# ARISE-Initiative/robosuite

Measured on NVIDIA H100. Metric: env-steps/sec (device-timed) Panda-Lift OSC_POSE @4096 envs per GPU, higher is better.
Workload: dtype f32

## Files before the change

### robosuite_b200/csrc/b2s_capi.cu

```cuda
#include "../../include/b2s.h"
#include "b2s_unit.cuh"
#include "b2s_snapshot.cuh"

#include <cmath>
#include <cstdio>
#include <cstdlib>
#include <cstring>
#include <map>
#include <algorithm>
#include <string>
#include <type_traits>
#include <vector>

static thread_local std::string g_err;
static int fail(int code, const std::string& msg) { g_err = msg; return code; }
#define CUDA_TRY(x) do { cudaError_t e_ = (x); if (e_ != cudaSuccess) return fail(B2S_ERR_CUDA, std::string(#x) + ": " + cudaGetErrorString(e_)); } while (0)

struct BlobRec { char name[48]; int32_t dtype, ndim, shape[4]; int64_t off, nbytes; };
struct Blob {
  const char* p; size_t n;
  const BlobRec* find(const char* name) const {
    int64_t cnt; memcpy(&cnt, p + 8, 8);
    const BlobRec* r = (const BlobRec*)(p + 16);
    for (int64_t i = 0; i < cnt; i++) if (!strcmp(r[i].name, name)) return r + i;
// ... 773 lines not shown
  CUDA_TRY(cudaMemsetAsync(st.cl_cnt + CL_CNT_STRIDE * gi, 0, CL_CNT_STRIDE * sizeof(int), q));
  for (int sub = 0; sub < nsub; sub++) {
    g.sub = sub;
    phase0_kernel<R><<<blocks0, s->wpb0 * 32, s->smem0, q>>>(phases, g);
    P1Cfg c{std::min(nG, cvx_blocks), ctrl_ext ? (g.nenv + OSC_TPB - 1) / OSC_TPB : 0, sub};
    int nAb = (nA + 31) / 32;
    if (c.nG + c.nC + nAb > 0) phase1_kernel<R><<<c.nG + c.nC + nAb, 32, p1smem, q>>>(action, g, c);
    if (s->tail_wide) tail_kernel<R, TAIL_WIDE_THREADS, true><<<blocks5, s->wpb5 * 32, s->smem5, q>>>(phases, nsub, action, g, s->stride5, s->stride5l, s->nlw5);
    else if (st.tail_sorted) tail_kernel<R, TAIL_THREADS, true><<<blocks5, s->wpb5 * 32, s->smem5, q>>>(phases, nsub, action, g, s->stride5, s->stride5l, s->nlw5);
    else tail_kernel<R, TAIL_THREADS, false><<<blocks5, s->wpb5 * 32, s->smem5, q>>>(phases, nsub, action, g, s->stride5, s->stride5l, s->nlw5);
  }
  CUDA_TRY(cudaGetLastError());
  return B2S_OK;
}

template <typename R> static int ensure_ws(b2s_sim* s, const DModel<R>& m, DState<R>& st) {
  if (!st.wsg) {
    R* p = nullptr;
    if (cudaMalloc(&p, (size_t)s->n_env * s->lay[LAY_ROW].total * sizeof(R)) != cudaSuccess) return fail(B2S_ERR_CUDA, "cudaMalloc(pipeline workspace) failed");
    cudaMemsetAsync(p, 0, (size_t)s->n_env * s->lay[LAY_ROW].total * sizeof(R), s->stream);
    s->allocs.push_back(p);
    st.wsg = p;
    size_t ne = (size_t)s->n_env;
    st.cl_cnt = dev_zeros<int>(s, CL_CNT_STRIDE * 64);
    st.tail_key = dev_zeros<int>(s, ne); st.tail_list = dev_zeros<int>(s, ne * TAIL_NKEY); st.tail_order = dev_zeros<int>(s, ne);
    s->arrays["tail_key"] = ArrayInfo{st.tail_key, B2S_I32, 1, {(int64_t)ne, 0, 0, 0}};
    s->arrays["tail_order"] = ArrayInfo{st.tail_order, B2S_I32, 1, {(int64_t)ne, 0, 0, 0}};
    st.cl_maxa = s->maxcon <= 32 ? 8 : (s->maxcon <= 48 ? 16 : CL_MAXA);
    st.cl_maxg = s->maxcon <= 32 ? 16 : CL_MAXG;
    st.cl_listA = dev_zeros<int>(s, ne * st.cl_maxa); st.cl_listG = dev_zeros<int>(s, ne * st.cl_maxg);
    st.cl_outA = dev_zeros<R>(s, ne * st.cl_maxa * CL_RECA); st.cl_outG = dev_zeros<R>(s, ne * st.cl_maxg * 8);
    st.cl_env = dev_zeros<int>(s, ne * CL_ENVW(st));
    st.gjk_cache = getenv("B2S_NO_GJK_CACHE") ? nullptr : dev_zeros<R>(s, ne * (size_t)m.npair * 3);
    s->action_buf = dev_zeros<R>(s, ne * 16);
#ifdef B2S_INSTR
    st.st_begin = dev_zeros<unsigned long long>(s, 64 * 32 * 8); st.st_end = dev_zeros<unsigned long long>(s, 64 * 32 * 8);
    st.stats = dev_zeros<int>(s, 512); st.cyc = dev_zeros<float>(s, ne * 32 * 8); st.solve_ls = dev_zeros<int>(s, ne);
    s->arrays["st_begin"] = ArrayInfo{st.st_begin, B2S_I64, 1, {64 * 32 * 8, 0, 0, 0}};
    s->arrays["st_end"] = ArrayInfo{st.st_end, B2S_I64, 1, {64 * 32 * 8, 0, 0, 0}};
    s->arrays["stats"] = ArrayInfo{st.stats, B2S_I32, 1, {512, 0, 0, 0}};
    s->arrays["cyc"] = ArrayInfo{st.cyc, B2S_F32, 3, {(int64_t)ne, 32, 8, 0}};
    st.slowlog = dev_zeros<int>(s, 64 * 12);
    s->arrays["slowlog"] = ArrayInfo{st.slowlog, B2S_I32, 2, {64, 12, 0, 0}};
    s->uq_prof = dev_zeros<unsigned long long>(s, 16);
    s->arrays["unit_prof"] = ArrayInfo{s->uq_prof, B2S_I64, 1, {16, 0, 0, 0}};
#endif
    s->dirty = 1;
    s->layout_version++;
  }
  return B2S_OK;
}

static int launch_pipeline(b2s_sim* s, int phases, int nsub, const void* action) {
  return with_real(s, [&](auto& m, auto& st) -> int {
    using R = real_of<decltype(m)>;
    { int rc0 = ensure_ws(s, m, st); if (rc0 != B2S_OK) return rc0; }
#ifdef B2S_INSTR
    cudaMemsetAsync(st.st_begin, 0xff, sizeof(unsigned long long) * 64 * 32 * 8, s->stream);
    cudaMemsetAsync(st.st_end, 0, sizeof(unsigned long long) * 64 * 32 * 8, s->stream);
#endif
    const bool osc = s->ctrl.kind == B2S_CTRL_OSC_POSE || s->ctrl.kind == B2S_CTRL_OSC_POSITION;
    if ((phases & PH_CTRL) && osc && s->ctrl_split) phases |= PH_CTRL_EXT;
    { int rc2 = rebuild_layouts(s); if (rc2 != B2S_OK) return rc2; }
    int rc = bind_constants(s);
    if (rc != B2S_OK) return rc;
    const int G = std::min(s->ngroups, s->n_env);
    while ((int)s->gstreams.size() < G) {
      cudaStream_t st2; cudaEvent_t ev;
      CUDA_TRY(cudaStreamCreateWithFlags(&st2, cudaStreamNonBlocking));
      CUDA_TRY(cudaEventCreateWithFlags(&ev, cudaEventDisableTiming));
      s->gstreams.push_back(st2); s->gevents.push_back(ev);
    }
    if (!s->in_event) CUDA_TRY(cudaEventCreateWithFlags(&s->in_event, cudaEventDisableTiming));
    const int launches_per_call = G * nsub * 3;
    const R* act_in = (const R*)action;
    if (action) {
// ... 761 lines not shown
```

### robosuite_b200/csrc/b2s_collide.cuh

```cuda
#pragma once
#include <cstdio>
#include "b2s_engine.cuh"

template <typename R>
struct Shape {
  int type;
  const R* pos;
  const R* mat;
  R size[3];
  const R* vert;
  int nvert;
};

template <typename R>
DEV void shape_from(const DModel<R>& m, const DState<R>& st, int env, int g, const R* gpos, const R* gmat, Shape<R>& s) {
  int k = m.geom_cgid[g];
  s.type = m.geom_type[g];
  s.pos = gpos + 3 * k;
  s.mat = gmat + 9 * k;
  const R* sz = geom_size_of(m, st, g, env);
  s.size[0] = sz[0]; s.size[1] = sz[1]; s.size[2] = sz[2];
  s.vert = nullptr; s.nvert = 0;
  if (s.type == G_MESH) {
    int id = m.geom_dataid[g];
// ... 407 lines not shown
    v3addscl(pos, pnt, nr, -R(0.5) * hh);
    cnt = put(out, cnt, maxn, pos, n, hh);
  }
  return cnt;
}

template <typename R> DEVN void support_w(const Shape<R>& s, R dx, R dy, R dz, R* out, int lane) {
  R l[3], pnt[3] = {0, 0, 0};
  const R dir[3] = {dx, dy, dz};
  m3mulTv(l, s.mat, dir);
  switch (s.type) {
    case G_BOX:
      pnt[0] = l[0] >= 0 ? s.size[0] : -s.size[0];
      pnt[1] = l[1] >= 0 ? s.size[1] : -s.size[1];
      pnt[2] = l[2] >= 0 ? s.size[2] : -s.size[2];
      break;
    case G_CYLINDER: {
      R nn = r_sqrt(l[0] * l[0] + l[1] * l[1]);
      if (nn > R(1e-12)) { pnt[0] = l[0] / nn * s.size[0]; pnt[1] = l[1] / nn * s.size[0]; }
      pnt[2] = l[2] >= 0 ? s.size[1] : -s.size[1];
      break;
    }
    case G_CAPSULE: pnt[2] = l[2] >= 0 ? s.size[1] : -s.size[1]; break;
    case G_ELLIPSOID: {
      R t[3] = {l[0] * s.size[0], l[1] * s.size[1], l[2] * s.size[2]};
      R nn = v3norm(t);
      if (nn > R(1e-12)) { pnt[0] = t[0] * s.size[0] / nn; pnt[1] = t[1] * s.size[1] / nn; pnt[2] = t[2] * s.size[2] / nn; }
      break;
    }
    case G_MESH: {
      R best = -Lim<R>::big();
      int bi = 0x7fffffff;
      const R* vt = s.vert;
      for (int i = lane; i < s.nvert; i += 32) {
        R v = vt[3 * i] * l[0] + vt[3 * i + 1] * l[1] + vt[3 * i + 2] * l[2];
        if (v > best) { best = v; bi = i; }
      }
      warp_argmax(best, bi);
      pnt[0] = vt[3 * bi]; pnt[1] = vt[3 * bi + 1]; pnt[2] = vt[3 * bi + 2];
      break;
    }
    default: break;
  }
  m3mulv(out, s.mat, pnt);
  v3add(out, out, s.pos);
}
template <typename R> DEV R shape_radius(const Shape<R>& s) { return (s.type == G_SPHERE || s.type == G_CAPSULE) ? s.size[0] : R(0); }

template <typename R> struct SV { R w[3], a[3], b[3]; };

template <typename R> DEV void sv_support(const Shape<R>& A, const Shape<R>& B, const R* dir, SV<R>& o, int lane) {
  const R dx = dir[0], dy = dir[1], dz = dir[2];
  support_w(A, dx, dy, dz, o.a, lane);
  support_w(B, -dx, -dy, -dz, o.b, lane);
  v3sub(o.w, o.a, o.b);
}

template <typename R> DEV void sx_load(const R* sx, int k, SV<R>& o) {
  const R* p = sx + 9 * k;
#pragma unroll
  for (int e = 0; e < 3; e++) { o.w[e] = p[e]; o.a[e] = p[3 + e]; o.b[e] = p[6 + e]; }
}
template <typename R> DEV void sx_store(R* sx, int k, const SV<R>& v, int lane) {
  __syncwarp();
  if (lane == 0) {
    R* p = sx + 9 * k;
#pragma unroll
    for (int e = 0; e < 3; e++) { p[e] = v.w[e]; p[3 + e] = v.a[e]; p[6 + e] = v.b[e]; }
  }
  __syncwarp();
// ... 71 lines not shown
    R so = orient3(w4[f0], w4[f1], w4[f2], zero);
    R sd = orient3(w4[f0], w4[f1], w4[f2], w4[op]);
    if (r_abs(sd) < tiny) outside = 1;
    if (r_abs(sd) >= tiny && so * sd > 0) continue;
    outside = 1;
    int tn, idx[3];
    R tl[3];
    tri_closest(w4[f0], w4[f1], w4[f2], tn, idx, tl);
    R pp[3] = {0, 0, 0};
#pragma unroll
    for (int k = 0; k < 3; k++)
      if (k < tn) {
        const int j = idx[k];
#pragma unroll
        for (int e = 0; e < 3; e++) pp[e] += (j == 0 ? w4[f0][e] : (j == 1 ? w4[f1][e] : w4[f2][e])) * tl[k];
      }
    R dd = v3dot(pp, pp);
    if (dd < bestd) {
      bestd = dd; bestn = tn;
      bi0 = idx[0] == 0 ? f0 : (idx[0] == 1 ? f1 : f2);
      bi1 = tn > 1 ? (idx[1] == 0 ? f0 : (idx[1] == 1 ? f1 : f2)) : 0;
      bi2 = tn > 2 ? (idx[2] == 0 ? f0 : (idx[2] == 1 ? f1 : f2)) : 0;
#pragma unroll
      for (int k = 0; k < 3; k++) bestlam[k] = tl[k];
    }
  }
  if (!outside) return 1;
  n = bestn;
  sx_select(sx, bestn, bi0, bi1, bi2, lane);
  for (int k = 0; k < bestn; k++) lam[k] = bestlam[k];
  return 0;
}

template <typename R>
DEVN int gjk(const Shape<R>& A, const Shape<R>& B, R* sx, int& ns, R& dist, R* wa, R* wb, R cutoff, int lane, R* cache = nullptr) {
  const R tol_vv = sizeof(R) == 4 ? R(1e-16) : R(1e-24);
  const R tol_rel = sizeof(R) == 4 ? R(1e-6) : R(1e-12);
  R v[3], nv[3];
  v3sub(v, A.pos, B.pos);
  if (v3dot(v, v) < R(1e-20)) v3set(v, R(1), R(0), R(0));
  if (cache) {
    R cv[3] = {cache[0], cache[1], cache[2]};
    if (v3dot(cv, cv) > R(1e-12)) v3copy(v, cv);
  }
  int n = 0;
  R lam[4] = {1, 0, 0, 0};
  v3scl(nv, v, R(-1));
  SV<R> w;
  sv_support(A, B, nv, w, lane);
  sx_store(sx, 0, w, lane);
  n = 1;
  if (cache && cutoff >= 0) {
    R vv0 = v3dot(v, v), vw0 = v3dot(v, w.w);
    if (vw0 > 0 && vw0 * vw0 > cutoff * cutoff * vv0) { dist = cutoff + 1; ns = 1; return 0; }
  }
  v3copy(v, w.w);
  const int max_it = sizeof(R) == 4 ? 32 : 64;
  for (int it = 0; it < max_it; it++) {
    R vv = v3dot(v, v);
    if (vv < tol_vv) { ns = n; if (cache && lane == 0) { cache[0] = 0; cache[1] = 0; cache[2] = 0; } return 1; }
    v3scl(nv, v, R(-1));
    sv_support(A, B, nv, w, lane);
    R vw = v3dot(v, w.w);
    if (cutoff >= 0 && vw > 0 && vw * vw > cutoff * cutoff * vv) {
      dist = cutoff + 1; ns = n;
      if (cache && lane == 0) { cache[0] = v[0]; cache[1] = v[1]; cache[2] = v[2]; }
      return 0;
    }
    if (vv - vw <= tol_rel * vv) break;
    int dup = 0;
    for (int k = 0; k < n; k++) {
      R e3[3];
      v3sub(e3, sx + 9 * k, w.w);
      if (v3dot(e3, e3) < tol_vv) dup = 1;
    }
    if (dup) break;
    sx_store(sx, n, w, lane);
    n++;
    if (n == 2) closest_seg(sx, n, lam, lane);
    else if (n == 3) closest_tri(sx, n, lam, lane);
    else if (closest_tet(sx, n, lam, lane)) { ns = 4; if (cache && lane == 0) { cache[0] = 0; cache[1] = 0; cache[2] = 0; } return 1; }
    v3set(v, R(0), R(0), R(0));
    for (int k = 0; k < n; k++) v3addscl(v, v, sx + 9 * k, lam[k]);
  }
  ns = n;
  dist = v3norm(v);
  if (cache && lane == 0) { cache[0] = v[0]; cache[1] = v[1]; cache[2] = v[2]; }
  v3set(wa, R(0), R(0), R(0));
  v3set(wb, R(0), R(0), R(0));
  for (int k = 0; k < n; k++) { v3addscl(wa, wa, sx + 9 * k + 3, lam[k]); v3addscl(wb, wb, sx + 9 * k + 6, lam[k]); }
  return 0;
// ... 159 lines not shown
  }
#ifdef B2S_INSTR
  if (lane == 0) { edges[64] = nV; edges[65] = nF; }
#endif
  if (bestf < 0) return -1;
  int fi = Fi[bestf];
  int ia = fi & 255, ib = (fi >> 8) & 255, ic = (fi >> 16) & 255;
  depth = Fn[4 * bestf + 3];
  normal[0] = Fn[4 * bestf]; normal[1] = Fn[4 * bestf + 1]; normal[2] = Fn[4 * bestf + 2];
  R pp[3], v0[3], v1[3], v2[3];
  v3scl(pp, normal, depth);
  const R *a = V + 9 * ia, *b = V + 9 * ib, *c = V + 9 * ic;
  v3sub(v0, b, a); v3sub(v1, c, a); v3sub(v2, pp, a);
  R d00 = v3dot(v0, v0), d01 = v3dot(v0, v1), d11 = v3dot(v1, v1), d20 = v3dot(v2, v0), d21 = v3dot(v2, v1);
  R den = d00 * d11 - d01 * d01;
  R bv = den != 0 ? (d11 * d20 - d01 * d21) / den : R(0), bw = den != 0 ? (d00 * d21 - d01 * d20) / den : R(0);
  R bu = 1 - bv - bw;
  for (int k = 0; k < 3; k++) {
    wa[k] = bu * a[3 + k] + bv * b[3 + k] + bw * c[3 + k];
    wb[k] = bu * a[6 + k] + bv * b[6 + k] + bw * c[6 + k];
  }
  __syncwarp();
  return 0;
}

template <typename R>
DEVN int convex_convex(const Shape<R>& A0, const Shape<R>& B0, R* out, int maxn, R* scratch, int lane, R* cache = nullptr,
                       int maxv = EPA_MAXV, int maxf = EPA_MAXF, R* stage = nullptr, int stage_cap = 0) {
  R* simplex = EPA_SIMPLEX(scratch, maxv, maxf);
  int ns = 0;
  R dist = 0, wa[3], wb[3], n[3], pos[3], pa[3], pb[3];
  Shape<R> A = A0, B = B0;
  R ra = shape_radius(A), rb = shape_radius(B);
  if (stage != nullptr) {
    __syncwarp();
    if (lane < 12) stage[lane] = lane < 3 ? A.pos[lane] : A.mat[lane - 3];
    else if (lane < 24) stage[lane] = lane < 15 ? B.pos[lane - 12] : B.mat[lane - 15];
    A.pos = stage; A.mat = stage + 3; B.pos = stage + 12; B.mat = stage + 15;
    stage += 24; stage_cap -= 24;
    __syncwarp();
    if (cache != nullptr) {
      R cv[3] = {cache[0], cache[1], cache[2]};
      if (v3dot(cv, cv) > R(1e-12)) {
        R nv[3] = {-cv[0], -cv[1], -cv[2]};
        SV<R> w0;
        sv_support(A, B, nv, w0, lane);
        R vv0 = v3dot(cv, cv), vw0 = v3dot(cv, w0.w), cut = ra + rb;
        if (vw0 > 0 && vw0 * vw0 > cut * cut * vv0) return 0;
      }
    }
    __syncwarp();
    int used = 0;
    if (A.nvert > 0 && 3 * A.nvert <= stage_cap) {
      for (int i = lane; i < 3 * A.nvert; i += 32) stage[i] = A.vert[i];
      A.vert = stage; used = (3 * A.nvert + 3) & ~3;
    }
    if (B.nvert > 0 && used + 3 * B.nvert <= stage_cap) {
      if (B.vert == A0.vert && A.vert == stage) B.vert = stage;
      else { for (int i = lane; i < 3 * B.nvert; i += 32) stage[used + i] = B.vert[i]; B.vert = stage + used; }
    }
    __syncwarp();
  }
#ifdef B2S_INSTR
  long long tg0 = clock64();
#endif
  int hit = gjk(A, B, simplex, ns, dist, wa, wb, ra + rb, lane, cache);
#ifdef B2S_INSTR
  if (stage != nullptr && lane == 0) {
    int* sp = reinterpret_cast<int*>(scratch + 9 * maxv + 4 * maxf) + maxf + 64;
    sp[2] = (int)(clock64() - tg0); sp[3] = hit; sp[0] = 0; sp[1] = 0; sp[4] = (A.vert == stage) | ((B.vert != B0.vert) << 1);
  }
#endif
  if (!hit) {
    if (ra + rb <= 0 || dist > ra + rb) return 0;
    v3sub(n, wb, wa);
    v3scl(n, n, R(1) / dist);
    v3addscl(pa, wa, n, ra);
    v3addscl(pb, wb, n, -rb);
    v3add(pos, pa, pb);
    v3scl(pos, pos, R(0.5));
    return put(out, 0, maxn, pos, n, dist - ra - rb);
  }
  R depth;
  if (epa(A, B, simplex, ns, depth, n, wa, wb, scratch, lane, maxv, maxf) != 0) return 0;
  v3addscl(pa, wa, n, ra);
  v3addscl(pb, wb, n, -rb);
  v3add(pos, pa, pb);
  v3scl(pos, pos, R(0.5));
  return put(out, 0, maxn, pos, n, -depth - ra - rb);
}

template <typename R> DEVN bool obb_overlap(const Eng<R> e, int g1, int g2) {
  const DModel<R>& m = e.model();
  int k1 = m.geom_cgid[g1], k2 = m.geom_cgid[g2];
  const R* M1 = e.p(e.lay().gmat) + 9 * k1; const R* M2 = e.p(e.lay().gmat) + 9 * k2;
  const R* a1 = geom_aabb_of(m, e.state(), g1, e.env); const R* a2 = geom_aabb_of(m, e.state(), g2, e.env);
  R c1[3], c2[3], t[3];
  R o1[3] = {a1[0], a1[1], a1[2]}, o2[3] = {a2[0], a2[1], a2[2]};
  m3mulv(t, M1, o1); v3add(c1, t, e.p(e.lay().gpos) + 3 * k1);
// ... 282 lines not shown
```

### robosuite_b200/csrc/b2s_pipeline.cuh

```cuda
#pragma once
#include "b2s_kernel.cuh"

DEV unsigned smem_u32(const void* p) { return (unsigned)__cvta_generic_to_shared(p); }
DEV void mbar_init(unsigned long long* bar) {
  asm volatile("mbarrier.init.shared::cta.b64 [%0], 1;" ::"r"(smem_u32(bar)));
  asm volatile("fence.mbarrier_init.release.cluster;" ::: "memory");
}
DEV void mbar_expect_tx(unsigned long long* bar, unsigned bytes) {
  asm volatile("mbarrier.arrive.expect_tx.shared::cta.b64 _, [%0], %1;" ::"r"(smem_u32(bar)), "r"(bytes) : "memory");
}
DEV void mbar_wait(unsigned long long* bar, unsigned parity) {
  asm volatile(
      "{\n"
      ".reg .pred p;\n"
      "WAIT_%=:\n"
      "mbarrier.try_wait.parity.shared::cta.b64 p, [%0], %1;\n"
      "@p bra DONE_%=;\n"
      "bra WAIT_%=;\n"
      "DONE_%=:\n"
      "}\n" ::"r"(smem_u32(bar)), "r"(parity) : "memory");
}
DEV void tma_load_1d(void* smem_dst, const void* gsrc, unsigned bytes, unsigned long long* bar) {
  asm volatile("cp.async.bulk.shared::cluster.global.mbarrier::complete_tx::bytes [%0], [%1], %2, [%3];" ::"r"(smem_u32(smem_dst)),
               "l"(gsrc), "r"(bytes), "r"(smem_u32(bar))
// ... 21 lines not shown
  __syncwarp();
  if (e.lane < io.nstore) {
    Region r = io.store[e.lane];
    tma_store_1d(row + r.goff, e.ws + r.off, (unsigned)r.len * sizeof(R));
    asm volatile("cp.async.bulk.commit_group;" ::: "memory");
    asm volatile("cp.async.bulk.wait_group 0;" ::: "memory");
  }
  __syncwarp();
}

struct Grp { int env0, nenv, gid, sub, slot; };
#define CLC(s, g) ((s).cl_cnt + CL_CNT_STRIDE * (g).gid)
#define CLK(s, g, sub) (CLC(s, g) + 8 + TAIL_NKEY * ((sub) & 1))

DEV int tail_cost_key(int niter, int nefc, bool large) {
  return large ? TAIL_NKEY - 1 : min(TAIL_NKEY - 2, (niter * (nefc + 24) + 2 * nefc) / 48);
}

#ifdef B2S_INSTR
DEV unsigned long long gtimer() { unsigned long long t; asm volatile("mov.u64 %0, %globaltimer;" : "=l"(t)); return t; }
#define INSTR_SLOT(g, kind) ((((g).gid & 63) * 32 + ((g).sub & 31)) * 8 + (kind))
#define INSTR_BEGIN(st, g, kind) if (threadIdx.x == 0 && (st).st_begin) atomicMin((st).st_begin + INSTR_SLOT(g, kind), gtimer());
#define INSTR_END(st, g, kind) if ((threadIdx.x & 31) == 0 && (st).st_end) atomicMax((st).st_end + INSTR_SLOT(g, kind), gtimer());
#else
#define INSTR_BEGIN(st, g, kind)
#define INSTR_END(st, g, kind)
#endif
#include "b2s_ctrlkernel.cuh"

struct P1Cfg { int nG, nC, sub; };

template <typename R> DEV R* gjk_cache_of(const DModel<R>& m, const DState<R>& s, int env, int pidx) {
  return s.gjk_cache ? s.gjk_cache + ((size_t)env * m.npair + pidx) * 3 : (R*)nullptr;
}

template <typename R> DEV void narrow_analytic_block(const Grp& g, int rb) {
  const DState<R>& s = cstate<R>(g.slot);
  const WSLayout& RL = c_lay[g.slot][LAY_ROW];
  int tid = rb * 32 + threadIdx.x;
  if (tid >= CLC(s, g)[0]) return;
  tid += g.env0 * s.cl_maxa;
  int code = s.cl_listA[tid];
  int env = code >> 12;
  const R* row = s.wsg + (size_t)env * RL.total;
  R buf[8 * CREC];
  const int n = narrow_pair_analytic(cmodel<R>(g.slot), s, env, code & 4095, row + RL.gpos, row + RL.gmat, buf);
  R* out = s.cl_outA + (size_t)tid * CL_RECA;
  out[0] = R(n);
  for (int k = 0; k < n * CREC; k++) out[1 + k] = buf[k];
}

template <typename R> DEV void narrow_convex_block(const Grp& g, unsigned char* smem_raw) {
  const DModel<R>& m = cmodel<R>(g.slot);
  const DState<R>& s = cstate<R>(g.slot);
  const WSLayout& RL = c_lay[g.slot][LAY_ROW];
  int lane = threadIdx.x & 31;
  R* scratch = reinterpret_cast<R*>(smem_raw);
  const int cnt = CLC(s, g)[1];
  while (true) {
    int item = 0;
    if (lane == 0) item = atomicAdd(CLC(s, g) + 3, 1);
    item = __shfl_sync(B2S_FULL, item, 0);
    if (item >= cnt) break;
    int wid = item + g.env0 * s.cl_maxg;
    int code = s.cl_listG[wid], env = code >> 12, pidx = code & 4095;
    const R* row = s.wsg + (size_t)env * RL.total;
    R buf[CREC];
    const int n = narrow_pair_convex(m, s, env, pidx, row + RL.gpos, row + RL.gmat, buf, scratch, gjk_cache_of(m, s, env, pidx),
                                     m.stage_cap > 0 ? scratch + EPA_AREA_WORDS(EPA_MAXV, EPA_MAXF) : (R*)nullptr, m.stage_cap, lane, true);
    if (lane == 0) {
      R* out = s.cl_outG + (size_t)wid * 8;
      out[0] = R(n);
      for (int k = 0; k < CREC; k++) out[1 + k] = n ? buf[k] : R(0);
    }
    __syncwarp();
  }
}

template <typename R>
__global__ void __launch_bounds__(32) phase1_kernel(const R* action, Grp g, P1Cfg c) {
  extern __shared__ __align__(16) unsigned char smem_raw[];
  const int b = blockIdx.x;
#ifdef B2S_INSTR
  const DState<R>& s = cstate<R>(g.slot);
  const int kind = b < c.nG ? 2 : (b < c.nG + c.nC ? 4 : 1);
  INSTR_BEGIN(s, g, kind)
#endif
  if (b < c.nG) narrow_convex_block<R>(g, smem_raw);
  else if (b < c.nG + c.nC) ctrl_osc_block<R>(g.sub, action, g.env0, g.nenv, g.gid, g.slot, smem_raw, b - c.nG);
  else narrow_analytic_block<R>(g, b - c.nG - c.nC);
#ifdef B2S_INSTR
  INSTR_END(s, g, kind)
#endif
}

template <typename R> DEVN int gather_contacts(Eng<R> e, int env, int& warn) {
  const DModel<R>& m = e.model();
  const DState<R>& s = e.state();
  const WSLayout& L = e.lay();
  int lane = e.lane;
  const int* tab = s.cl_env + (size_t)env * CL_ENVW(s);
  int na = tab[0], ng = tab[1], nc = na + ng;
  const int IT = 3;
  int nchunk = (nc + 31) >> 5;
  int pairv[IT], slotv[IT], isgv[IT], cntv[IT], offv[IT];
#pragma unroll
  for (int it = 0; it < IT; it++) {
// ... 43 lines not shown
  __syncwarp();
  finish_contacts(e, total);
  return total;
}


template <typename R> DEV int phase0_env(Eng<R>& e, int env, int& na, int& ng) {
  const DModel<R>& m = e.model();
  const DState<R>& s = e.state();
  const WSLayout& L = e.lay();
  const int lane = e.lane;
  const size_t E = env;
  e.env = env;
  load_row(e.p(L.qpos), s.qpos + E * m.nq, m.nq, lane);
  load_row(e.p(L.qvel), s.qvel + E * m.nv, m.nv, lane);
  __syncwarp();
  const int was_reset = e.kinematics();
  if (was_reset) {
    for (int i = lane; i < m.nq; i += 32) s.qpos[E * m.nq + i] = e.p(L.qpos)[i];
    for (int i = lane; i < m.nv; i += 32) { s.qvel[E * m.nv + i] = 0; s.qacc[E * m.nv + i] = 0; s.qacc_ws[E * m.nv + i] = 0; }
    if (lane == 0) s.time[env] = 0;
    __syncwarp();
  }
  e.velocity();
  e.crb();
  int* cand = e.pi(L.scratch);
  int warn = was_reset;
  cull_pairs(e, cand, cand + 96, s.cl_maxa, s.cl_maxg, na, ng);
  if (na > s.cl_maxa) { na = s.cl_maxa; warn |= 4; }
  if (ng > s.cl_maxg) { ng = s.cl_maxg; warn |= 4; }
  return warn;
}

template <typename R> DEV void phase0_publish(const Eng<R>& e, int env, int na, int ng, int warn, int baseA, int baseG, bool worklist) {
  const DState<R>& s = e.state();
  const WSLayout& L = e.lay();
  const WSLayout& RL = c_lay[e.slot][LAY_ROW];
  const int lane = e.lane;
  const size_t E = env;
  const int* cand = e.pi(L.scratch);
  const int* cand_g = cand + 96;
  int* tab = s.cl_env + E * CL_ENVW(s);
  if (lane == 0) { tab[0] = na; tab[1] = ng; }
  for (int i = lane; i < na; i += 32) {
    if (worklist) s.cl_listA[baseA + i] = (env << 12) | cand[i];
    tab[2 + 2 * i] = cand[i]; tab[3 + 2 * i] = baseA + i;
  }
  for (int i = lane; i < ng; i += 32) {
    if (worklist) s.cl_listG[baseG + i] = (env << 12) | cand_g[i];
    tab[2 + 2 * (s.cl_maxa + i)] = cand_g[i]; tab[3 + 2 * (s.cl_maxa + i)] = baseG + i;
  }
  R* row = s.wsg + E * RL.total;
  if (lane == 0) reinterpret_cast<int*>(row + RL.hdr)[2] = warn;
  __syncwarp();
  ws_store(e, row, c_pio[e.slot][PIO_P0]);
}

#define TAIL_NCON(pk) ((pk) & 255)
#define TAIL_WARN(pk) (((pk) >> 8) & 255)
#define TAIL_NEFC(pk) (((pk) >> 16) & 0x3fff)
#define TAIL_OVF(pk) ((pk) >> 30)
template <typename R> DEV int tail_rows(Eng<R>& e, int env, unsigned long long* bar, unsigned& parity) {
  const DModel<R>& m = e.model();
  const DState<R>& s = e.state();
  const WSLayout& L = e.lay();
  const WSLayout& RL = c_lay[e.slot][LAY_ROW];
  const int lane = e.lane;
  const bool tiered = L.mc < m.maxcon || L.me < m.maxefc;
  const size_t E = env;
  e.env = env;
  const R* row = s.wsg + E * RL.total;
  const int warn = reinterpret_cast<const int*>(row + RL.hdr)[2];
  ws_load(e, row, c_pio[e.slot][e.lid == LAY_TL ? PIO_TL : PIO_TS], bar, parity);
  load_row(e.p(L.qpos), s.qpos + E * m.nq, m.nq, lane);
  load_row(e.p(L.qvel), s.qvel + E * m.nv, m.nv, lane);
  load_row(e.p(L.ctrl), s.ctrl + E * m.nu, m.nu, lane);
  load_row(e.p(L.qacc_ws), s.qacc_ws + E * m.nv, m.nv, lane);
  __syncwarp();
  int wl = 0;
  const int ncon = gather_contacts(e, env, wl);
  const int nefc = (tiered && (wl & 4)) ? 0 : make_constraint(e, ncon, wl);
  wl = warp_or_i(wl);
  const int ovf = (tiered && (wl & 12)) ? 1 : 0;
// ... 31 lines not shown
  R time = s.time[env];
  if (!(phases & PH_NOINTEGRATE)) {
    { int eb = e.euler(&time); if (eb & 32) warn |= 32; else if (eb) warn |= 2; }
  }
  if ((phases & PH_OBS) && e.ccfg().obs_dim > 0 && sub == nsub - 1) {
    ws_load(e, s.wsg + (size_t)env * c_lay[e.slot][LAY_ROW].total, c_pio[e.slot][e.lid == LAY_TL ? PIO_TL_LATE : PIO_TS_LATE], bar, parity);
    write_obs(e, env, (phases & PH_NOINTEGRATE) != 0);
    write_task(e, env, ncon);
  }
  store_state(e, env, time, warn);
}

constexpr int P0_THREADS = 256, P0_BLOCKS = 2;
constexpr int TAIL_THREADS = 256, TAIL_BLOCKS = 2;
constexpr int TAIL_WIDE_THREADS = 512;

template <typename R>
__global__ void __launch_bounds__(P0_THREADS, P0_BLOCKS) phase0_kernel(int phases, Grp g) {
  const DState<R>& s = cstate<R>(g.slot);
  const WSLayout& L = c_lay[g.slot][LAY_P0];
  extern __shared__ __align__(16) unsigned char smem_raw[];
  R* smem = reinterpret_cast<R*>(smem_raw);
  int warp = threadIdx.x >> 5, lane = threadIdx.x & 31, wpb = blockDim.x >> 5;
  int env = blockIdx.x * wpb + warp;
  INSTR_BEGIN(s, g, 0)
#ifdef B2S_INSTR
  long long instr_t0 = clock64();
#endif
  if (env >= g.nenv) return;
  env += g.env0;
  Eng<R> e(smem + (size_t)warp * L.total, lane, g.slot, LAY_P0);
  int na, ng;
  const int warn = phase0_env(e, env, na, ng);
  int baseA = 0, baseG = 0;
  if (lane == 0) {
    if (na) baseA = g.env0 * s.cl_maxa + atomicAdd(CLC(s, g), na);
    if (ng) baseG = g.env0 * s.cl_maxg + atomicAdd(CLC(s, g) + 1, ng);
    if (s.tail_sorted) {
      const int k = s.tail_key[env];
      s.tail_list[(size_t)g.env0 * TAIL_NKEY + k * g.nenv + atomicAdd(CLK(s, g, g.sub) + k, 1)] = env;
    }
  }
  baseA = __shfl_sync(B2S_FULL, baseA, 0);
  baseG = __shfl_sync(B2S_FULL, baseG, 0);
  phase0_publish(e, env, na, ng, warn, baseA, baseG, true);
#ifdef B2S_INSTR
  if (lane == 0 && s.cyc) s.cyc[((size_t)env * 32 + (g.sub & 31)) * 8] = (float)(clock64() - instr_t0);
#endif
  INSTR_END(s, g, 0)
}

template <typename R> DEV int tail_env_at(const Grp& g, int p, int lane) {
  const DState<R>& s = cstate<R>(g.slot);
  const int wpb = blockDim.x >> 5;
  if (TAIL_SOLO * wpb <= g.nenv) {
    const int b = p / wpb, w = p - b * wpb;
    if (b >= TAIL_SOLO) p -= TAIL_SOLO * (wpb - 1);
    else p = w == 0 ? b : g.nenv - 1 - (b * (wpb - 1) + w - 1);
  }
  const int cnt = lane < TAIL_NKEY ? CLK(s, g, g.sub)[TAIL_NKEY - 1 - lane] : 0;
  int incl = cnt;
#pragma unroll
  for (int d = 1; d < TAIL_NKEY; d <<= 1) {
    const int v = __shfl_up_sync(B2S_FULL, incl, d);
    if (lane >= d) incl += v;
  }
  const int c = __ffs(__ballot_sync(B2S_FULL, incl > p)) - 1;
  const int rank = p - __shfl_sync(B2S_FULL, incl - cnt, c);
  return s.tail_list[(size_t)g.env0 * TAIL_NKEY + (TAIL_NKEY - 1 - c) * g.nenv + rank];
}

template <typename R, bool SORTED>
DEVN int tail_env(R* area, int lane, int lid, Grp g, int env, int nsub, int phases, const R* action, unsigned long long* bar, unsigned& parity) {
  const int sub = g.sub;
  if (SORTED && lid == LAY_TS) {
    const int p = env;
    env = tail_env_at<R>(g, p, lane);
    if (lane == 0) cstate<R>(g.slot).tail_order[g.env0 + p] = env;
// ... 6 lines not shown
  const int pk = tail_rows(e, env, bar, parity);
  if (TAIL_OVF(pk)) return 1;
  const int ncon = TAIL_NCON(pk), nefc = TAIL_NEFC(pk);
  int warn = TAIL_WARN(pk);
  if ((phases & PH_CTRL) && !(phases & PH_CTRL_EXT)) tail_ctrl(e, env, sub, action);
  warn |= tail_accel(e);
  int niter;
  warn |= tail_newton(e, nefc, ncon, &niter);
  if (SORTED && lane == 0) e.state().tail_key[env] = tail_cost_key(niter, nefc, lid == LAY_TL);
  tail_finish(e, env, sub, nsub, phases, ncon, warn, bar, parity);
#ifdef B2S_INSTR
  if (lane == 0 && s.cyc) {
    float* c = s.cyc + ((size_t)env * 32 + (sub & 31)) * 8;
    c[1] = (float)(clock64() - instr_t0);
    c[2] = (float)niter; c[3] = (float)s.solve_ls[env]; c[4] = (float)nefc; c[5] = (float)ncon;
    c[6] = lid == LAY_TL ? 1.f : 0.f; c[7] = (float)blockIdx.x;
  }
  if (lane == 0 && s.stats) { atomicAdd(s.stats + 32 + min(ncon, 128), 1); atomicAdd(s.stats + 176 + min(nefc, 320), 1); if (lid == LAY_TL) atomicAdd(s.stats + 19, 1); }
#endif
  return 0;
}

template <typename R, int THREADS, bool SORTED>
__global__ void __launch_bounds__(THREADS, THREADS == TAIL_WIDE_THREADS ? 1 : TAIL_BLOCKS) tail_kernel(int phases, int nsub, const R* action, Grp g, int stride, int stride_l, int nlw) {
  const DState<R>& s = cstate<R>(g.slot);
  extern __shared__ __align__(16) unsigned char smem_raw[];
  R* smem = reinterpret_cast<R*>(smem_raw);
  const int warp = threadIdx.x >> 5, lane = threadIdx.x & 31, wpb = blockDim.x >> 5;
  INSTR_BEGIN(s, g, 3)
  __shared__ unsigned long long mbar[32];
  __shared__ int ovf[32];
  if (blockIdx.x == 0 && warp == 0) {
    int* c = CLC(s, g);
    if (lane == 0) { c[0] = 0; c[1] = 0; c[3] = 0; }
    if (lane < TAIL_NKEY) CLK(s, g, g.sub + 1)[lane] = 0;
  }
  if (lane == 0) mbar_init(&mbar[warp]);
  __syncwarp();
  unsigned parity = 0;
  const int p = blockIdx.x * wpb + warp;
  int o = -1;
  if (p < g.nenv && tail_env<R, SORTED>(smem + (size_t)warp * stride, lane, LAY_TS, g, SORTED ? p : g.env0 + p, nsub, phases, action, &mbar[warp], parity)) o = p;
  if (lane == 0) ovf[warp] = o;
  asm volatile("fence.proxy.async.shared::cta;" ::: "memory");
  __syncthreads();
  if (warp < nlw)
    for (int k = warp; k < wpb; k += nlw)
      if (ovf[k] >= 0)
        tail_env<R, SORTED>(smem + (size_t)warp * stride_l, lane, LAY_TL, g, SORTED ? s.tail_order[g.env0 + ovf[k]] : g.env0 + ovf[k], nsub, phases, action, &mbar[warp], parity);
  INSTR_END(s, g, 3)
}
```

### robosuite_b200/csrc/b2s_types.cuh

```cuda
#pragma once
#include <cuda_runtime.h>
#include <stdint.h>

#define B2S_FULL 0xffffffffu
#define B2S_MOV 8

enum { JNT_FREE = 0, JNT_BALL = 1, JNT_SLIDE = 2, JNT_HINGE = 3 };
enum { G_PLANE = 0, G_HFIELD, G_SPHERE, G_CAPSULE, G_ELLIPSOID, G_CYLINDER, G_BOX, G_MESH };
enum { C_FRICTION = 1, C_LIMIT = 3, C_FRICTIONLESS = 5, C_ELLIPTIC = 7 };
enum { DK_FREE_T = 0, DK_FREE_R = 1, DK_SLIDE = 2, DK_HINGE = 3 };

enum {
  PH_STEP1 = 1,
  PH_STEP2 = 2,
  PH_NOINTEGRATE = 4,
  PH_EXPORT = 8,
  PH_CTRL = 16,
  PH_CTRL_EXT = 512,
  PH_OBS = 64
};

template <typename R>
struct DModel {
  int nq, nv, nu, nbody, njnt, ngeom, nsite, npair, ncg, nment, maxdepth, maxcon, maxefc, nmocap, nfl, nlim, hc_stride, max_treesize;
// ... 37 lines not shown
  R* obs;
  R* wsg;
  int* cl_cnt;
  int cl_maxa, cl_maxg;
  int* cl_listA;
  int* cl_listG;
  R* cl_outA;
  R* cl_outG;
  R* gjk_cache;
  int* cl_env;
  int tail_sorted;
  int* tail_key;
  int* tail_list;
  int* tail_order;
  int* obs_fresh;
  int n_ov, ov_body[4];
  R* ov_pos[4];
  R* ov_quat[4];
  int n_mg, n_mb;
  short mg_id[B2S_MOV], mb_id[B2S_MOV];
  R *mg_size, *mg_fric, *mg_rbound, *mg_aabb;
  R *mb_mass, *mb_inertia;
  R *mg_solref, *mg_solimp;
  R *dof_iw, *body_iw, *mean_inertia;
  R *dof_damp, *dof_arm, *dof_floss;
  R* task_vec;
  R* task_out;
  unsigned long long* st_begin;
  unsigned long long* st_end;
  int* stats;
  float* cyc;
  int* solve_ls;
  int* slowlog;
};

struct WSLayout {
  int qpos, qvel, qacc, qacc_ws, ctrl;
  int xpos, xquat, xmat, xipos;
  int cdof, cdofdot, cinert, cvel, frne, ffl;
  int M, H;
  int bias, passive, qact, qsmooth, qaccs, qcon;
  int gpos, gmat, spos, smat;
  int c_pos, c_frame, c_dist, c_fric, c_solref, c_solimp, c_mu, c_int;
  int J, e_D, e_R, e_aref, e_jar, e_jv, e_force, e_floss, e_int;
  int Ma, grad, search, Mv;
  int scratch, scratch_size;
  int fused_stride;
  int hdr;
  int total;
  int mc, me;
};

#define B2S_NSLOT 8
enum { LAY_FULL = 0, LAY_P0 = 1, LAY_TS = 2, LAY_TL = 3, LAY_ROW = 4, B2S_NLAY = 5 };

struct Region { int off, goff, len, dyn; };
enum { PIO_P0 = 0, PIO_TS = 1, PIO_TS_LATE = 2, PIO_TL = 3, PIO_TL_LATE = 4, B2S_NPIO = 5 };
#define CL_MAXA 64
#define CL_MAXG 32
#define CL_RECA 58
#define CL_ENVW(s) (2 + 2 * ((s).cl_maxa + (s).cl_maxg))
#define TAIL_NKEY 16
#define TAIL_SOLO 2
#define CL_CNT_STRIDE (8 + 2 * TAIL_NKEY)
#define B2S_MAXREG 12
struct PhaseIO { int nload, nstore, load_words, load_dyn; Region load[B2S_MAXREG], store[B2S_MAXREG]; };
// ... 32 lines not shown
```

### robosuite_b200/csrc/b2s_unit.cuh

```cuda
#pragma once
#include "b2s_pipeline.cuh"

struct UnitQ {
  int* ring;
  int* ovf_ring;
  int* ctr;
  int total, n_large, wpb_large;
  int stride, stride_large;
#ifdef B2S_INSTR
  unsigned long long* prof;
#endif
};

DEV int ld_acquire_gpu(const int* p) { int v; asm volatile("ld.acquire.gpu.global.s32 %0, [%1];" : "=r"(v) : "l"(p) : "memory"); return v; }
DEV int ld_relaxed_gpu(const int* p) { int v; asm volatile("ld.relaxed.gpu.global.s32 %0, [%1];" : "=r"(v) : "l"(p) : "memory"); return v; }
DEV void st_release_gpu(int* p, int v) { asm volatile("st.release.gpu.global.s32 [%0], %1;" ::"l"(p), "r"(v) : "memory"); }
DEV void fence_proxy_async_all() { asm volatile("fence.proxy.async;" ::: "memory"); }

template <typename R> __global__ void unit_init_kernel(UnitQ q, int n_env) {
  int i = blockIdx.x * blockDim.x + threadIdx.x;
  if (i < q.total) { q.ring[i] = i < n_env ? i : -1; q.ovf_ring[i] = -1; }
  if (i < 8) q.ctr[i] = i == 1 ? n_env : 0;
}

template <typename R> __global__ void unit_check_kernel(UnitQ q, int slot) {
  const DState<R>& s = cstate<R>(slot);
  if (q.ctr[7] == 0) return;
  for (int i = blockIdx.x * blockDim.x + threadIdx.x; i < s.n_env; i += gridDim.x * blockDim.x) s.warn[i] |= 64;
}


template <typename R> DEVN int unit_phase0(R* area, int lane, int slot, int env) {
  const DState<R>& s = cstate<R>(slot);
  Eng<R> e(area, lane, slot, LAY_P0);
  int na, ng;
  const int warn = phase0_env(e, env, na, ng);
  phase0_publish(e, env, na, ng, warn, env * s.cl_maxa, env * s.cl_maxg, false);
  return na | (ng << 16);
}

template <typename R> DEVN void unit_narrow(R* area, int area_words, int lane, int slot, int env, int na, int ng) {
  const DModel<R>& m = cmodel<R>(slot);
  const DState<R>& s = cstate<R>(slot);
  const WSLayout& RL = c_lay[slot][LAY_ROW];
  size_t E = env;
  const R* row = s.wsg + E * RL.total;
  const int* tab = s.cl_env + E * CL_ENVW(s);
  for (int base = 0; base < na; base += 32) {
    int i = base + lane;
    if (i < na) {
      R buf[8 * CREC];
      const int n = narrow_pair_analytic(m, s, env, tab[2 + 2 * i], row + RL.gpos, row + RL.gmat, buf);
      R* out = s.cl_outA + (E * s.cl_maxa + i) * CL_RECA;
      out[0] = R(n);
      for (int k = 0; k < n * CREC; k++) out[1 + k] = buf[k];
    }
  }
  __syncwarp();
  const int epa_words = EPA_AREA_WORDS(EPA_MAXV, EPA_MAXF), stage_cap = area_words - epa_words;
  for (int i = 0; i < ng; i++) {
    const int pidx = tab[2 + 2 * (s.cl_maxa + i)];
    R buf[CREC];
    const int n = narrow_pair_convex(m, s, env, pidx, row + RL.gpos, row + RL.gmat, buf, area, gjk_cache_of(m, s, env, pidx),
                                     stage_cap >= 64 ? area + epa_words : (R*)nullptr, stage_cap >= 64 ? stage_cap : 0, lane, false);
    if (lane == 0) {
      R* out = s.cl_outG + (E * s.cl_maxg + i) * 8;
      out[0] = R(n);
      for (int k = 0; k < CREC; k++) out[1 + k] = n ? buf[k] : R(0);
    }
    __syncwarp();
// ... 185 lines not shown
```

Before: 336,200.

## Split convex narrowphase worklist into heavy and light pairs, reuse GJK first support

Convex pairs without a cached separating direction are classed as heavy and written to the front of the worklist, while light pairs are written from the back. Workers pull heavy items first, so long GJK/EPA jobs start early and the tail is shorter. The separation-test support point is now stored as the GJK starting simplex, so it is not computed twice. The mesh support loop is unrolled four ways with independent per-lane maxima, and instrumentation-only per-item records are added. Risks are an extra counter and ballots in phase0, and a publish path that now assumes at most 32 convex candidates per env.

```diff
diff --git a/robosuite_b200/csrc/b2s_capi.cu b/robosuite_b200/csrc/b2s_capi.cu
--- a/robosuite_b200/csrc/b2s_capi.cu
+++ b/robosuite_b200/csrc/b2s_capi.cu
@@ -829,6 +829,9 @@
     st.cl_outA = dev_zeros<R>(s, ne * st.cl_maxa * CL_RECA); st.cl_outG = dev_zeros<R>(s, ne * st.cl_maxg * 8);
     st.cl_env = dev_zeros<int>(s, ne * CL_ENVW(st));
     st.gjk_cache = getenv("B2S_NO_GJK_CACHE") ? nullptr : dev_zeros<R>(s, ne * (size_t)m.npair * 3);
+    s->arrays["cl_listG"] = ArrayInfo{st.cl_listG, B2S_I32, 1, {(int64_t)(ne * st.cl_maxg), 0, 0, 0}};
+    s->arrays["cl_env"] = ArrayInfo{st.cl_env, B2S_I32, 2, {(int64_t)ne, CL_ENVW(st), 0, 0}};
+    if (st.gjk_cache && m.npair > 0) s->arrays["gjk_cache"] = ArrayInfo{st.gjk_cache, DT<R>::code, 3, {(int64_t)ne, m.npair, 3, 0}};
     s->action_buf = dev_zeros<R>(s, ne * 16);
 #ifdef B2S_INSTR
     st.st_begin = dev_zeros<unsigned long long>(s, 64 * 32 * 8); st.st_end = dev_zeros<unsigned long long>(s, 64 * 32 * 8);
@@ -839,6 +842,8 @@
     s->arrays["cyc"] = ArrayInfo{st.cyc, B2S_F32, 3, {(int64_t)ne, 32, 8, 0}};
     st.slowlog = dev_zeros<int>(s, 64 * 12);
     s->arrays["slowlog"] = ArrayInfo{st.slowlog, B2S_I32, 2, {64, 12, 0, 0}};
+    st.cvx_rec = dev_zeros<long long>(s, 32 * ne * st.cl_maxg * 8);
+    s->arrays["cvx_rec"] = ArrayInfo{st.cvx_rec, B2S_I64, 3, {32, (int64_t)(ne * st.cl_maxg), 8, 0}};
     s->uq_prof = dev_zeros<unsigned long long>(s, 16);
     s->arrays["unit_prof"] = ArrayInfo{s->uq_prof, B2S_I64, 1, {16, 0, 0, 0}};
 #endif
diff --git a/robosuite_b200/csrc/b2s_collide.cuh b/robosuite_b200/csrc/b2s_collide.cuh
--- a/robosuite_b200/csrc/b2s_collide.cuh
+++ b/robosuite_b200/csrc/b2s_collide.cuh
@@ -463,10 +463,29 @@
       R best = -Lim<R>::big();
       int bi = 0x7fffffff;
       const R* vt = s.vert;
-      for (int i = lane; i < s.nvert; i += 32) {
-        R v = vt[3 * i] * l[0] + vt[3 * i + 1] * l[1] + vt[3 * i + 2] * l[2];
-        if (v > best) { best = v; bi = i; }
+      R b4[4] = {best, best, best, best};
+      int i4[4] = {bi, bi, bi, bi};
+      int i = lane;
+      for (; i + 96 < s.nvert; i += 128) {
+#pragma unroll
+        for (int k = 0; k < 4; k++) {
+          const int j = i + 32 * k;
+          R v = vt[3 * j] * l[0] + vt[3 * j + 1] * l[1] + vt[3 * j + 2] * l[2];
+          if (v > b4[k]) { b4[k] = v; i4[k] = j; }
+        }
       }
+#pragma unroll
+      for (int k = 0; k < 3; k++) {
+        const int j = i + 32 * k;
+        if (j < s.nvert) {
+          R v = vt[3 * j] * l[0] + vt[3 * j + 1] * l[1] + vt[3 * j + 2] * l[2];
+          if (v > b4[k]) { b4[k] = v; i4[k] = j; }
+        }
+      }
+      best = b4[0]; bi = i4[0];
+#pragma unroll
+      for (int k = 1; k < 4; k++)
+        if (b4[k] > best || (b4[k] == best && i4[k] < bi)) { best = b4[k]; bi = i4[k]; }
       warp_argmax(best, bi);
       pnt[0] = vt[3 * bi]; pnt[1] = vt[3 * bi + 1]; pnt[2] = vt[3 * bi + 2];
       break;
@@ -604,10 +623,7 @@
   return 0;
 }
 
-template <typename R>
-DEVN int gjk(const Shape<R>& A, const Shape<R>& B, R* sx, int& ns, R& dist, R* wa, R* wb, R cutoff, int lane, R* cache = nullptr) {
-  const R tol_vv = sizeof(R) == 4 ? R(1e-16) : R(1e-24);
-  const R tol_rel = sizeof(R) == 4 ? R(1e-6) : R(1e-12);
+template <typename R> DEV int gjk_first(const Shape<R>& A, const Shape<R>& B, const R* cache, R cutoff, SV<R>& w, int lane) {
   R v[3], nv[3];
   v3sub(v, A.pos, B.pos);
   if (v3dot(v, v) < R(1e-20)) v3set(v, R(1), R(0), R(0));
@@ -615,20 +631,40 @@
     R cv[3] = {cache[0], cache[1], cache[2]};
     if (v3dot(cv, cv) > R(1e-12)) v3copy(v, cv);
   }
-  int n = 0;
-  R lam[4] = {1, 0, 0, 0};
   v3scl(nv, v, R(-1));
-  SV<R> w;
   sv_support(A, B, nv, w, lane);
-  sx_store(sx, 0, w, lane);
-  n = 1;
   if (cache && cutoff >= 0) {
     R vv0 = v3dot(v, v), vw0 = v3dot(v, w.w);
-    if (vw0 > 0 && vw0 * vw0 > cutoff * cutoff * vv0) { dist = cutoff + 1; ns = 1; return 0; }
+    if (vw0 > 0 && vw0 * vw0 > cutoff * cutoff * vv0) return 1;
+  }
+  return 0;
+}
+
+template <typename R>
+DEVN int gjk(const Shape<R>& A, const Shape<R>& B, R* sx, int& ns, R& dist, R* wa, R* wb, R cutoff, int lane, R* cache = nullptr,
+             bool warm = false) {
+  const R tol_vv = sizeof(R) == 4 ? R(1e-16) : R(1e-24);
+  const R tol_rel = sizeof(R) == 4 ? R(1e-6) : R(1e-12);
+  R v[3], nv[3];
+  int n = 1;
+  R lam[4] = {1, 0, 0, 0};
+#ifdef B2S_INSTR
+  int* const it_note = reinterpret_cast<int*>(sx + 36);
+  if (lane == 0) *it_note = 0;
+#endif
+  SV<R> w;
+  if (warm) sx_load(sx, 0, w);
+  else {
+    const int sep = gjk_first(A, B, cache, cutoff, w, lane);
+    sx_store(sx, 0, w, lane);
+    if (sep) { dist = cutoff + 1; ns = 1; return 0; }
   }
   v3copy(v, w.w);
   const int max_it = sizeof(R) == 4 ? 32 : 64;
   for (int it = 0; it < max_it; it++) {
+#ifdef B2S_INSTR
+    if (lane == 0) *it_note = it + 1;
+#endif
     R vv = v3dot(v, v);
     if (vv < tol_vv) { ns = n; if (cache && lane == 0) { cache[0] = 0; cache[1] = 0; cache[2] = 0; } return 1; }
     v3scl(nv, v, R(-1));
@@ -854,6 +890,7 @@
   R dist = 0, wa[3], wb[3], n[3], pos[3], pa[3], pb[3];
   Shape<R> A = A0, B = B0;
   R ra = shape_radius(A), rb = shape_radius(B);
+  bool warm = false;
   if (stage != nullptr) {
     __syncwarp();
     if (lane < 12) stage[lane] = lane < 3 ? A.pos[lane] : A.mat[lane - 3];
@@ -862,14 +899,10 @@
     stage += 24; stage_cap -= 24;
     __syncwarp();
     if (cache != nullptr) {
-      R cv[3] = {cache[0], cache[1], cache[2]};
-      if (v3dot(cv, cv) > R(1e-12)) {
-        R nv[3] = {-cv[0], -cv[1], -cv[2]};
-        SV<R> w0;
-        sv_support(A, B, nv, w0, lane);
-        R vv0 = v3dot(cv, cv), vw0 = v3dot(cv, w0.w), cut = ra + rb;
-        if (vw0 > 0 && vw0 * vw0 > cut * cut * vv0) return 0;
-      }
+      SV<R> w0;
+      if (gjk_first(A, B, cache, ra + rb, w0, lane)) return 0;
+      sx_store(simplex, 0, w0, lane);
+      warm = true;
     }
     __syncwarp();
     int used = 0;
@@ -886,7 +919,7 @@
 #ifdef B2S_INSTR
   long long tg0 = clock64();
 #endif
-  int hit = gjk(A, B, simplex, ns, dist, wa, wb, ra + rb, lane, cache);
+  int hit = gjk(A, B, simplex, ns, dist, wa, wb, ra + rb, lane, cache, warm);
 #ifdef B2S_INSTR
   if (stage != nullptr && lane == 0) {
     int* sp = reinterpret_cast<int*>(scratch + 9 * maxv + 4 * maxf) + maxf + 64;
diff --git a/robosuite_b200/csrc/b2s_pipeline.cuh b/robosuite_b200/csrc/b2s_pipeline.cuh
--- a/robosuite_b200/csrc/b2s_pipeline.cuh
+++ b/robosuite_b200/csrc/b2s_pipeline.cuh
@@ -77,6 +77,11 @@
 
 template <typename R> DEV R* gjk_cache_of(const DModel<R>& m, const DState<R>& s, int env, int pidx) {
   return s.gjk_cache ? s.gjk_cache + ((size_t)env * m.npair + pidx) * 3 : (R*)nullptr;
+}
+template <typename R> DEV bool cvx_heavy(const R* cache) {
+  if (cache == nullptr) return false;
+  R cv[3] = {cache[0], cache[1], cache[2]};
+  return !(v3dot(cv, cv) > R(1e-12));
 }
 
 template <typename R> DEV void narrow_analytic_block(const Grp& g, int rb) {
@@ -101,15 +106,21 @@
   const WSLayout& RL = c_lay[g.slot][LAY_ROW];
   int lane = threadIdx.x & 31;
   R* scratch = reinterpret_cast<R*>(smem_raw);
-  const int cnt = CLC(s, g)[1];
+  const int nl = CLC(s, g)[1], nh = CLC(s, g)[2];
   while (true) {
     int item = 0;
     if (lane == 0) item = atomicAdd(CLC(s, g) + 3, 1);
     item = __shfl_sync(B2S_FULL, item, 0);
-    if (item >= cnt) break;
-    int wid = item + g.env0 * s.cl_maxg;
+    if (item >= nh + nl) break;
+    int wid = (item < nh ? item : g.nenv * s.cl_maxg - 1 - (item - nh)) + g.env0 * s.cl_maxg;
     int code = s.cl_listG[wid], env = code >> 12, pidx = code & 4095;
     const R* row = s.wsg + (size_t)env * RL.total;
+#ifdef B2S_INSTR
+    int* const sp = reinterpret_cast<int*>(scratch + 9 * EPA_MAXV + 4 * EPA_MAXF) + EPA_MAXF + 64;
+    const unsigned long long t0 = gtimer();
+    if (lane == 0) sp[3] = -1;
+    __syncwarp();
+#endif
     R buf[CREC];
     const int n = narrow_pair_convex(m, s, env, pidx, row + RL.gpos, row + RL.gmat, buf, scratch, gjk_cache_of(m, s, env, pidx),
                                      m.stage_cap > 0 ? scratch + EPA_AREA_WORDS(EPA_MAXV, EPA_MAXF) : (R*)nullptr, m.stage_cap, lane, true);
@@ -118,6 +129,21 @@
       out[0] = R(n);
       for (int k = 0; k < CREC; k++) out[1 + k] = n ? buf[k] : R(0);
     }
+#ifdef B2S_INSTR
+    if (lane == 0 && s.cvx_rec) {
+      long long* r = s.cvx_rec + ((size_t)(g.sub & 31) * s.n_env * s.cl_maxg + wid) * 8;
+      int g1, g2;
+      pair_geoms(m, pidx, g1, g2);
+      const int t1 = m.geom_type[g1], t2 = m.geom_type[g2];
+      const long long v1 = t1 == G_MESH ? m.mesh_vertnum[m.geom_dataid[g1]] : 0, v2 = t2 == G_MESH ? m.mesh_vertnum[m.geom_dataid[g2]] : 0;
+      const int gjk_it = *reinterpret_cast<const int*>(EPA_SIMPLEX(scratch, EPA_MAXV, EPA_MAXF) + 36);
+      const int outcome = sp[3] < 0 ? 0 : (sp[3] ? 2 : 1);
+      r[0] = (long long)t0; r[1] = (long long)gtimer(); r[2] = item; r[3] = blockIdx.x;
+      r[4] = t1 | (t2 << 4) | (v1 << 8) | (v2 << 32);
+      r[5] = outcome | ((outcome ? gjk_it : 0) << 4) | ((outcome == 2 ? sp[0] : 0) << 16);
+      r[6] = item < nh; r[7] = code;
+    }
+#endif
     __syncwarp();
   }
 }
@@ -227,7 +253,7 @@
   return warn;
 }
 
-template <typename R> DEV void phase0_publish(const Eng<R>& e, int env, int na, int ng, int warn, int baseA, int baseG, bool worklist) {
+template <typename R> DEV void phase0_publish(const Eng<R>& e, int env, int na, int ng, int warn, int baseA, int slotG, bool worklist) {
   const DState<R>& s = e.state();
   const WSLayout& L = e.lay();
   const WSLayout& RL = c_lay[e.slot][LAY_ROW];
@@ -241,9 +267,9 @@
     if (worklist) s.cl_listA[baseA + i] = (env << 12) | cand[i];
     tab[2 + 2 * i] = cand[i]; tab[3 + 2 * i] = baseA + i;
   }
-  for (int i = lane; i < ng; i += 32) {
-    if (worklist) s.cl_listG[baseG + i] = (env << 12) | cand_g[i];
-    tab[2 + 2 * (s.cl_maxa + i)] = cand_g[i]; tab[3 + 2 * (s.cl_maxa + i)] = baseG + i;
+  if (lane < ng) {
+    if (worklist) s.cl_listG[slotG] = (env << 12) | cand_g[lane];
+    tab[2 + 2 * (s.cl_maxa + lane)] = cand_g[lane]; tab[3 + 2 * (s.cl_maxa + lane)] = slotG;
   }
   R* row = s.wsg + E * RL.total;
   if (lane == 0) reinterpret_cast<int*>(row + RL.hdr)[2] = warn;
@@ -341,18 +367,24 @@
   Eng<R> e(smem + (size_t)warp * L.total, lane, g.slot, LAY_P0);
   int na, ng;
   const int warn = phase0_env(e, env, na, ng);
-  int baseA = 0, baseG = 0;
+  const bool heavy = lane < ng && cvx_heavy(gjk_cache_of(cmodel<R>(g.slot), s, env, e.pi(L.scratch)[96 + lane]));
+  const unsigned hm = __ballot_sync(B2S_FULL, heavy), lm = __ballot_sync(B2S_FULL, lane < ng && !heavy);
+  int baseA = 0, baseH = 0, baseL = 0;
   if (lane == 0) {
     if (na) baseA = g.env0 * s.cl_maxa + atomicAdd(CLC(s, g), na);
-    if (ng) baseG = g.env0 * s.cl_maxg + atomicAdd(CLC(s, g) + 1, ng);
+    if (hm) baseH = atomicAdd(CLC(s, g) + 2, __popc(hm));
+    if (lm) baseL = atomicAdd(CLC(s, g) + 1, __popc(lm));
     if (s.tail_sorted) {
       const int k = s.tail_key[env];
       s.tail_list[(size_t)g.env0 * TAIL_NKEY + k * g.nenv + atomicAdd(CLK(s, g, g.sub) + k, 1)] = env;
     }
   }
   baseA = __shfl_sync(B2S_FULL, baseA, 0);
-  baseG = __shfl_sync(B2S_FULL, baseG, 0);
-  phase0_publish(e, env, na, ng, warn, baseA, baseG, true);
+  baseH = __shfl_sync(B2S_FULL, baseH, 0);
+  baseL = __shfl_sync(B2S_FULL, baseL, 0);
+  const unsigned below = (1u << lane) - 1;
+  const int slotG = g.env0 * s.cl_maxg + (heavy ? baseH + __popc(hm & below) : g.nenv * s.cl_maxg - 1 - (baseL + __popc(lm & below)));
+  phase0_publish(e, env, na, ng, warn, baseA, slotG, true);
 #ifdef B2S_INSTR
   if (lane == 0 && s.cyc) s.cyc[((size_t)env * 32 + (g.sub & 31)) * 8] = (float)(clock64() - instr_t0);
 #endif
@@ -425,7 +457,7 @@
   __shared__ int ovf[32];
   if (blockIdx.x == 0 && warp == 0) {
     int* c = CLC(s, g);
-    if (lane == 0) { c[0] = 0; c[1] = 0; c[3] = 0; }
+    if (lane == 0) { c[0] = 0; c[1] = 0; c[2] = 0; c[3] = 0; }
     if (lane < TAIL_NKEY) CLK(s, g, g.sub + 1)[lane] = 0;
   }
   if (lane == 0) mbar_init(&mbar[warp]);
diff --git a/robosuite_b200/csrc/b2s_types.cuh b/robosuite_b200/csrc/b2s_types.cuh
--- a/robosuite_b200/csrc/b2s_types.cuh
+++ b/robosuite_b200/csrc/b2s_types.cuh
@@ -93,6 +93,7 @@
   float* cyc;
   int* solve_ls;
   int* slowlog;
+  long long* cvx_rec;
 };
 
 struct WSLayout {
diff --git a/robosuite_b200/csrc/b2s_unit.cuh b/robosuite_b200/csrc/b2s_unit.cuh
--- a/robosuite_b200/csrc/b2s_unit.cuh
+++ b/robosuite_b200/csrc/b2s_unit.cuh
@@ -35,7 +35,7 @@
   Eng<R> e(area, lane, slot, LAY_P0);
   int na, ng;
   const int warn = phase0_env(e, env, na, ng);
-  phase0_publish(e, env, na, ng, warn, env * s.cl_maxa, env * s.cl_maxg, false);
+  phase0_publish(e, env, na, ng, warn, env * s.cl_maxa, env * s.cl_maxg + lane, false);
   return na | (ng << 16);
 }
 
```

Result: faster. 343,700 (median of 6 runs) (+2.2%).
